# nv-tlabs/STRIVE

Measured on AMD Instinct MI355X. Metric: adv-optim agent*timesteps/sec (decoder fwd+bwd), higher is better.
Workload: dtype f32

## Files before the change

strive_amd/csrc/capi.hip:

```cpp
#include "common.h"
#include <stdarg.h>
#include <stddef.h>

static thread_local char g_err[512] = "";

void strive_set_error(const char* fmt, ...) {
    va_list ap;
    va_start(ap, fmt);
    vsnprintf(g_err, sizeof(g_err), fmt, ap);
    va_end(ap);
}

extern "C" const char* strive_last_error(void) { return g_err; }
extern "C" int strive_abi_version(void) { return STRIVE_ABI_VERSION; }

namespace {
struct OptionDesc { const char* name; size_t off; int def; int lo, hi; };
#define STRIVE_OPT(field, def, lo, hi) {#field, offsetof(StriveTuning, field), def, lo, hi}
const OptionDesc g_options[] = {
    STRIVE_OPT(cnn_small_batch, 96, 0, 1 << 20),
    STRIVE_OPT(cnn_chunk, 512, 8, 1024),
    STRIVE_OPT(cnn_tail_s, 0, 0, 4),
    STRIVE_OPT(conv_ws, 1, 0, 1),
    STRIVE_OPT(conv_wsx, 1, 0, 1),
    STRIVE_OPT(conv_ws_dbg, 0, 0, 255),
    STRIVE_OPT(scene_kernels, 1, 0, 1),
    STRIVE_OPT(scene_tiles, 1, 0, 1),
    STRIVE_OPT(scene_prof, 0, 0, 1),
    STRIVE_OPT(scene_split, 12, 0, 64),
    STRIVE_OPT(scene_fwd_k, -1, -1, 4),
    STRIVE_OPT(sweep_step, -1, -1, 4),
    STRIVE_OPT(train_overlap, 1, 0, 1),
    STRIVE_OPT(train_overlap_rows, 256, 1, 1 << 20),
    STRIVE_OPT(wgrad_atomics, 0, 0, 1),
    STRIVE_OPT(dgrad_igemm, 0, 0, 1),
    STRIVE_OPT(wgrad_igemm, 0, 0, 1),
    STRIVE_OPT(wgrad_tile, 0, 0, 1),
    STRIVE_OPT(wgrad_dbg, 0, 0, 255),
    STRIVE_OPT(planner_prof, 0, 0, 1),
    STRIVE_OPT(planner_dbg, 0, 0, 65535),
};
#undef STRIVE_OPT
constexpr int N_OPTIONS = (int)(sizeof(g_options) / sizeof(g_options[0]));
StriveTuning make_defaults() {
    StriveTuning t;
    for (int i = 0; i < N_OPTIONS; ++i) *reinterpret_cast<int*>(reinterpret_cast<char*>(&t) + g_options[i].off) = g_options[i].def;
    return t;
// ... 29 lines not shown
```

strive_amd/csrc/common.h:

```cpp
#pragma once
#include <hip/hip_runtime.h>
#include <atomic>
#include <stdint.h>
#include <stdio.h>
#include <string.h>
#include "../../include/strive_hip.h"

#define STRIVE_WAVE 64

void strive_set_error(const char* fmt, ...);

struct StriveTuning {
    int cnn_small_batch, cnn_chunk, cnn_tail_s, conv_ws, conv_wsx, conv_ws_dbg;
    int scene_kernels, scene_tiles, scene_prof, scene_split, scene_fwd_k, sweep_step;
    int train_overlap, train_overlap_rows;
    int wgrad_atomics, dgrad_igemm, wgrad_igemm, wgrad_tile, wgrad_dbg;
    int planner_prof;
    int planner_dbg;
};
StriveTuning& strive_tuning();

#define STRIVE_CHECK_ARG(cond, msg)                                   \
    do {                                                              \
        if (!(cond)) {                                                \
            strive_set_error("%s: %s", __func__, msg);                \
            return -1;                                                \
        }                                                             \
    } while (0)

#define STRIVE_CHECK_LAUNCH()                                                             \
    do {                                                                                  \
        hipError_t e__ = hipGetLastError();                                               \
        if (e__ != hipSuccess) {                                                          \
            strive_set_error("%s: kernel launch failed: %s", __func__, hipGetErrorString(e__)); \
            return -2;                                                                    \
        }                                                                                 \
// ... 86 lines not shown
```

strive_amd/csrc/map_cnn.hip:

```cpp
#include "common.h"
#include "crop_dev.h"
#include <type_traits>

typedef float f32x4 __attribute__((ext_vector_type(4)));
typedef float f32x16 __attribute__((ext_vector_type(16)));

#define GN_EPS 1e-5

struct GNStats { double sum, sq; };

__device__ __forceinline__ void gn_moments(const GNStats* __restrict__ st, int n, int nparts, double count, float& mean,
                                           float& rstd) {
    double s = 0.0, q = 0.0;
    for (int i = 0; i < nparts; ++i) {
        s += st[(size_t)n * nparts + i].sum;
        q += st[(size_t)n * nparts + i].sq;
    }
    const double m = s / count;
    double var = q / count - m * m;
    var = var < 0.0 ? 0.0 : var;
    mean = (float)m;
    rstd = (float)(1.0 / sqrt(var + GN_EPS));
}

// ... 210 lines not shown
    static constexpr int PT = PT_;
    static constexpr bool ROWS2 = ROWS2_;
    static constexpr int TILE_ROWS = ROWS2 ? 2 : 1;
    static constexpr int WGS_PER_CU = WGS_PER_CU_;
    static constexpr int NT = 256, NW = 4, TH = NW * PT * TILE_ROWS, TW = ROWS2 ? 16 : 32;
    static constexpr int CBW = CBW_, COUT_WG = 32 * CBW, CSPLIT = COUT / COUT_WG;
    static constexpr int PASS_CH = 8, NPASS = CIN / PASS_CH;
    static constexpr int ITH = 2 * TH + KS - 2, ITW = 2 * TW + KS - 2, HW = (ITW + 1) / 2;
    static constexpr int HALF_B = HW * 16, ROW_B = 2 * HALF_B, PIECE_B = ITH * ROW_B;
    static constexpr int NPIECE = 2;
    static constexpr int IN_B = (NPIECE * PIECE_B + 255) / 256 * 256;
    static constexpr int NKS = (KS * KS + 1) / 2;
    static constexpr int WSTEP_B = CBW * 2 * 64 * 16;
    static constexpr int TILES_X = (OH + TW - 1) / TW, TILES_Y = (OH + TH - 1) / TH;
    static constexpr int NPART_OUT = TILES_X * TILES_Y * CSPLIT;
    static constexpr int UNITS = ITH * ITW, UITERS = (UNITS + NT - 1) / NT;
    static constexpr size_t LDS_BYTES = (size_t)IN_B + 3 * WSTEP_B + (size_t)CIN * 8 + NW * 16 + 16 + COUT_WG * 4;
    static constexpr size_t WFRAG_BYTES = (size_t)NPASS * NKS * (COUT / 32) * 2048;
    static_assert(CIN % PASS_CH == 0 && COUT % COUT_WG == 0 && CIN <= NT, "channel tiling");
    static_assert(LDS_BYTES * WGS_PER_CU <= 160 * 1024, "LDS budget of the residency target");
    static_assert((KS == 5 && NKS == 13) || (KS == 3 && NKS == 5), "tap orders exist for 5x5 and 3x3 windows");
    static_assert(WSTEP_B == 16 * 128 * CBW && WSTEP_B / 16 <= NT, "weight step = one 16-byte piece for each of the first 128 CBW threads");
    static constexpr int W_UPFRONT = (WGS_PER_CU >= 3 && NKS > 8) ? 7 : NKS, W_LATE_AT = 2;
};

typedef float split_f32x2 __attribute__((ext_vector_type(2)));
typedef _Float16 split_f16x2v __attribute__((ext_vector_type(2)));
__device__ __forceinline__ void split_f16x2(const float v[8], uint4& p0, uint4& p1) {
    uint32_t h[4], l[4];
#pragma unroll
    for (int i = 0; i < 4; ++i) {
        const split_f32x2 v2 = {v[2 * i], v[2 * i + 1]};
        const split_f16x2v a = __builtin_convertvector(v2, split_f16x2v);
        const float r0 = v[2 * i] - (float)a[0];
        const float r1 = v[2 * i + 1] - (float)a[1];
        const split_f32x2 r2 = {r0, r1};
        const split_f16x2v c = __builtin_convertvector(r2, split_f16x2v);
        __builtin_memcpy(&h[i], &a, 4);
        __builtin_memcpy(&l[i], &c, 4);
    }
    p0 = make_uint4(h[0], h[1], h[2], h[3]);
    p1 = make_uint4(l[0], l[1], l[2], l[3]);
}

template <class Cfg, bool TIMING = false, int DBG = 0>
__global__ __launch_bounds__(Cfg::NT, Cfg::WGS_PER_CU) void conv_bf6_kernel(const float* __restrict__ in, const GNStats* __restrict__ st_in,
                                                                const float* __restrict__ gn_g, const float* __restrict__ gn_b,
                                                                const uint32_t* __restrict__ wfrag, const float* __restrict__ bias,
                                                                float* __restrict__ out, GNStats* __restrict__ st_out, int N,
                                                                float xscale, float unscale,
                                                                unsigned long long* __restrict__ tprof = nullptr) {
    long long tstamp[8];
    int nstamp = 0;
    auto stamp = [&]() { if (TIMING) tstamp[nstamp++] = clock64(); };
    stamp();
    constexpr int CIN = Cfg::CIN, COUT = Cfg::COUT, IH = Cfg::IH, OH = Cfg::OH, NT = Cfg::NT;
    constexpr int TH = Cfg::TH, TW = Cfg::TW, ITW = Cfg::ITW, PT = Cfg::PT;
    HIP_DYNAMIC_SHARED(float, smem)
    unsigned char* s_in = reinterpret_cast<unsigned char*>(smem);
    unsigned char* s_w = s_in + Cfg::IN_B;
    float* s_gn = (float*)(s_w + 3 * Cfg::WSTEP_B);
    double* s_red = (double*)(s_gn + 2 * CIN);
    float* s_mr = (float*)(s_red + 2 * Cfg::NW);
    float* s_bias = s_mr + 4;

    const int tid = threadIdx.x, lane = tid & 63, wave = tid >> 6;
    const int h = lane >> 5, j = lane & 31;
    int bx, by, n;
    {
        const unsigned T = gridDim.x * gridDim.y;
        const unsigned lin = blockIdx.x + gridDim.x * (blockIdx.y + gridDim.y * blockIdx.z);
        const unsigned q = lin >> 3, tile = q % T;
        n = (int)(8u * (q / T) + (lin & 7u));
        bx = (int)(tile % gridDim.x);
        by = (int)(tile / gridDim.x);
        if (n >= N) return;
    }
    const int tile_x = bx % Cfg::TILES_X, cb = bx / Cfg::TILES_X;
// ... 207 lines not shown
    const double lsum = wave_sum_d(dsum), lsq = wave_sum_d(dsq);
    if (lane == 0) { s_red[2 * wave] = lsum; s_red[2 * wave + 1] = lsq; }
    __syncthreads();
    if (tid == 0) {
        double a = 0.0, b = 0.0;
        for (int w = 0; w < Cfg::NW; ++w) { a += s_red[2 * w]; b += s_red[2 * w + 1]; }
        GNStats& o = st_out[(size_t)n * Cfg::NPART_OUT + (by * Cfg::TILES_X + tile_x) * Cfg::CSPLIT + cb];
        o.sum = a;
        o.sq = b;
    }
    stamp();
    if (TIMING && tid == 0) {
        atomicAdd(tprof, 1ull);
        for (int k = 0; k + 1 < nstamp; ++k) atomicAdd(tprof + 1 + k, (unsigned long long)(tstamp[k + 1] - tstamp[k]));
    }
}

template <class Cfg>
struct WsCfg {
    static constexpr int NCONS_W = 8, NT = 1024, NPROD = 512;
    static constexpr int UITERS = (Cfg::UNITS + NPROD - 1) / NPROD;
    static constexpr int W_B = Cfg::NPASS * Cfg::NKS * Cfg::WSTEP_B;
    static constexpr size_t LDS_BYTES = 2 * (size_t)Cfg::IN_B + W_B + 2 * (size_t)Cfg::CIN * 8 + 2 * 8 * 16 + 64 + Cfg::COUT * 4;
    static_assert(Cfg::CBW == 1 && Cfg::CSPLIT == 1 && Cfg::OUT_OCT && !Cfg::ROWS2 && Cfg::TH == NCONS_W, "built for conv2's shape");
    static_assert(LDS_BYTES <= 160 * 1024, "LDS budget");
};

template <class Cfg>
struct WsUnits {
    int t_begin, nunit;
    __device__ __forceinline__ void tile(int u, int& n, int& ty, int& tx, int& pass) const {
        constexpr int TPS = Cfg::TILES_X * Cfg::TILES_Y;
        const int t = t_begin + u / Cfg::NPASS;
        pass = u - (u / Cfg::NPASS) * Cfg::NPASS;
        n = t / TPS;
        const int r = t - n * TPS;
        tx = r / Cfg::TILES_Y;
        ty = r - tx * Cfg::TILES_Y;
    }
};

template <class Cfg>
__device__ __forceinline__ void ws_producer(const float* __restrict__ in, const GNStats* __restrict__ st_in, const float* __restrict__ gn_g,
                                         const float* __restrict__ gn_b, float xscale, unsigned char* s_in, float* s_gn,
                                         WsUnits<Cfg> un, int dbg, unsigned long long* __restrict__ tprof) {
    using W = WsCfg<Cfg>;
    constexpr int CIN = Cfg::CIN, IH = Cfg::IH, TH = Cfg::TH, TW = Cfg::TW, ITW = Cfg::ITW;
// ... 253 lines not shown
struct WxCfg {
    static constexpr int NCW = Cfg::NW, GW = Cfg::NW, NPW = NPW_, NT = 64 * (NCW + NPW + 1), NPROD = 64 * NPW;
    static constexpr int NSUB = Cfg::NKS > 7 ? 2 : 1;
    static constexpr int SUB_STEPS = (Cfg::NKS + NSUB - 1) / NSUB;
    static constexpr int WSUB_B = SUB_STEPS * Cfg::WSTEP_B;
    static constexpr int WCHUNKS = WSUB_B / 1024;
    static constexpr int UITERS = (Cfg::UNITS + NPROD - 1) / NPROD;
    static constexpr size_t LDS_BYTES = 2 * (size_t)Cfg::IN_B + 2 * (size_t)WSUB_B + 2 * (size_t)Cfg::CIN * 8 + 2 * GW * 16 + Cfg::COUT * 4 + 64;
    static_assert(Cfg::CSPLIT == 1 && Cfg::OUT_OCT && Cfg::NW == 4, "one workgroup computes all output channels of its tile");
    static_assert(LDS_BYTES <= 160 * 1024, "LDS budget");
    static_assert(NT <= 1024, "waves");
};

template <class Cfg, class W>
__device__ __forceinline__ void wx_producer(const float* __restrict__ in, const GNStats* __restrict__ st_in, const float* __restrict__ gn_g,
                                         const float* __restrict__ gn_b, float xscale, unsigned char* s_in, float* s_gn, WsUnits<Cfg> un,
                                         int dbg) {
    constexpr int CIN = Cfg::CIN, IH = Cfg::IH, TH = Cfg::TH, TW = Cfg::TW, ITW = Cfg::ITW;
    const int tid = threadIdx.x, lane = tid & 63;
    const int wave = __builtin_amdgcn_readfirstlane(tid >> 6);
    const int ptid = tid - 64 * W::NCW;
    const int nunit = un.nunit;
    float4 raw0[W::UITERS][2], raw1[W::UITERS][2];
    auto issue_loads = [&](int u, float4 (&raw)[W::UITERS][2]) {
        int n, ty, tx, pass;
        un.tile(u, n, ty, tx, pass);
        const float* in_n = in + (size_t)n * IH * IH * CIN;
        const int iy0 = 2 * ty * TH, ix0 = 2 * tx * TW;
#pragma unroll
        for (int k = 0; k < W::UITERS; ++k) {
            int idx = ptid + k * W::NPROD;
            idx = idx < Cfg::UNITS ? idx : Cfg::UNITS - 1;
            const int col = idx % ITW, r = idx / ITW;
            int iy = iy0 + r, ix = ix0 + col;
            iy = iy < IH ? iy : IH - 1;
            ix = ix < IH ? ix : IH - 1;
            const float4* src = reinterpret_cast<const float4*>(in_n + (((size_t)pass * IH + iy) * IH + ix) * 8);
            raw[k][0] = src[0];
            raw[k][1] = src[1];
        }
    };
    auto sample_moments = [&](int n) {
        double ps = 0.0, pq = 0.0;
        for (int i = lane; i < Cfg::NPART_IN; i += 64) {
            ps += st_in[(size_t)n * Cfg::NPART_IN + i].sum;
            pq += st_in[(size_t)n * Cfg::NPART_IN + i].sq;
        }
        ps = wave_sum_d(ps);
        pq = wave_sum_d(pq);
        const double cnt = (double)CIN * IH * IH;
        const double mu = ps / cnt;
        double var = pq / cnt - mu * mu;
        var = var < 0.0 ? 0.0 : var;
        const float mean = (float)mu, rstd = (float)(1.0 / sqrt(var + GN_EPS));
        if (lane < CIN) {
            const float sc = rstd * gn_g[lane];
            float* g = s_gn + (n & 1) * CIN * 2;
            g[2 * lane] = sc * xscale;
            g[2 * lane + 1] = (gn_b[lane] - mean * sc) * xscale;
        }
    };
    auto stage = [&](int u, const float4 (&raw)[W::UITERS][2], int chunk) {
        int n, ty, tx, pass;
        un.tile(u, n, ty, tx, pass);
        const int iy0 = 2 * ty * TH, ix0 = 2 * tx * TW;
        unsigned char* buf = s_in + (u & 1) * Cfg::IN_B;
        const float4* gn = reinterpret_cast<const float4*>(s_gn + (n & 1) * CIN * 2 + 2 * pass * Cfg::PASS_CH);
        const float4 g0 = gn[0], g1 = gn[1], g2 = gn[2], g3 = gn[3];
#pragma unroll
        for (int k = 0; k < W::UITERS; ++k) {
            if (chunk >= 0 && (k * W::NSUB) / W::UITERS != chunk) continue;
            const int idx = ptid + k * W::NPROD;
            if (idx < Cfg::UNITS) {
                const int col = idx % ITW, r = idx / ITW;
                const int iy = iy0 + r, ix = ix0 + col;
                float v[8];
#pragma unroll
                for (int e = 0; e < 8; ++e) v[e] = 0.f;
                if (iy < IH && ix < IH) {
                    const float4 a = raw[k][0], b = raw[k][1];
                    v[0] = fmaxf(fmaf(a.x, g0.x, g0.y), 0.f);
                    v[1] = fmaxf(fmaf(a.y, g0.z, g0.w), 0.f);
                    v[2] = fmaxf(fmaf(a.z, g1.x, g1.y), 0.f);
                    v[3] = fmaxf(fmaf(a.w, g1.z, g1.w), 0.f);
                    v[4] = fmaxf(fmaf(b.x, g2.x, g2.y), 0.f);
                    v[5] = fmaxf(fmaf(b.y, g2.z, g2.w), 0.f);
                    v[6] = fmaxf(fmaf(b.z, g3.x, g3.y), 0.f);
                    v[7] = fmaxf(fmaf(b.w, g3.z, g3.w), 0.f);
                }
                uint4 p0, p1;
                split_f16x2(v, p0, p1);
                unsigned char* dst = buf + r * Cfg::ROW_B + (col & 1) * Cfg::HALF_B + (col >> 1) * 16;
                *reinterpret_cast<uint4*>(dst) = p0;
                *reinterpret_cast<uint4*>(dst + Cfg::PIECE_B) = p1;
            }
        }
// ... 47 lines not shown
        for (int i = 0; i < W::WCHUNKS; ++i) w[i] = src[(i < nchunk ? i : nchunk - 1) * 64 + lane];
#pragma unroll
        for (int i = 0; i < W::WCHUNKS; ++i)
            if (i < nchunk) dst[i * 64 + lane] = w[i];
    };
    const int K = nunit * W::NSUB;
    __syncthreads();
    fill(0);
    __syncthreads();
    for (int k = 1; k <= K; ++k) {
        if (k < K && !(dbg & 8)) fill(k);
        __syncthreads();
    }
}

template <class Cfg, class W>
__device__ __forceinline__ void wx_consumer(const unsigned char* s_in, const unsigned char* s_w, double* s_red, const float* s_bias,
                                         float* __restrict__ out, GNStats* __restrict__ st_out, float unscale, WsUnits<Cfg> un, int dbg) {
    constexpr int COUT = Cfg::COUT, OH = Cfg::OH, TH = Cfg::TH, TW = Cfg::TW, NKS = Cfg::NKS, NPASS = Cfg::NPASS, PT = Cfg::PT, CBW = Cfg::CBW;
    const int tid = threadIdx.x, lane = tid & 63;
    const int wave = __builtin_amdgcn_readfirstlane(tid >> 6);
    const int h = lane >> 5, j = lane & 31;
    const int nunit = un.nunit;
    f32x16 acc[CBW][PT];
    const int gwave = wave;
    const int prow = Cfg::ROWS2 ? (j >> 4) : 0, pcol = Cfg::ROWS2 ? (j & 15) : j;
    const int lane_base = (2 * (Cfg::TILE_ROWS * PT * gwave + prow)) * Cfg::ROW_B + pcol * 16;

    auto matrix_sub = [&](int u, auto HC) {
        constexpr int HS = decltype(HC)::value;
        constexpr int S0 = HS * W::SUB_STEPS, S1 = (S0 + W::SUB_STEPS) < NKS ? (S0 + W::SUB_STEPS) : NKS;
        int n, ty, tx, pass;
        un.tile(u, n, ty, tx, pass);
        const unsigned char* buf = s_in + (u & 1) * Cfg::IN_B;
        const unsigned char* wbuf = s_w + ((u * W::NSUB + HS) & 1) * W::WSUB_B;
        if (pass == 0 && HS == 0) {
#pragma unroll
            for (int c = 0; c < CBW; ++c)
#pragma unroll
                for (int i = 0; i < PT; ++i)
#pragma unroll
                    for (int r = 0; r < 16; ++r) acc[c][i][r] = 0.f;
        }
        f16x8 fa[2][CBW][2], fb[2][PT][2];
        auto load_frags = [&](int t, int set) {
            int ky, kx;
            if (Cfg::KS == 5) {
                if (t < 10) { ky = t >> 1; kx = (t & 1) + 2 * h; }
                else { ky = 2 * (t - 10) + h; kx = 4; ky = ky > 4 ? 4 : ky; }
            } else {
                if (t < 3) { ky = t; kx = 2 * h; }
                else if (t == 3) { ky = h; kx = 1; }
                else { ky = 2; kx = 1; }
            }
            const int off = ky * Cfg::ROW_B + (kx & 1) * Cfg::HALF_B + (kx >> 1) * 16;
            const unsigned char* wb = wbuf + (t - S0) * Cfg::WSTEP_B + lane * 16;
#pragma unroll
            for (int c = 0; c < CBW; ++c)
#pragma unroll
                for (int pl = 0; pl < 2; ++pl) fa[set][c][pl] = *reinterpret_cast<const f16x8*>(wb + (c * 2 + pl) * 1024);
#pragma unroll
            for (int i = 0; i < PT; ++i)
#pragma unroll
                for (int pl = 0; pl < 2; ++pl)
                    fb[set][i][pl] = *reinterpret_cast<const f16x8*>(buf + pl * Cfg::PIECE_B + 2 * Cfg::TILE_ROWS * i * Cfg::ROW_B + lane_base + off);
        };
        load_frags(S0, 0);
#pragma unroll
        for (int s = S0; s < S1; ++s) {
            const int cur = (s - S0) & 1;
            if (s + 1 < S1) load_frags(s + 1, cur ^ 1);
            constexpr int TA[3] = {1, 0, 0}, TB[3] = {0, 1, 0};
#pragma unroll
            for (int term = 0; term < 3; ++term)
#pragma unroll
                for (int c = 0; c < CBW; ++c)
#pragma unroll
                    for (int i = 0; i < PT; ++i)
                        acc[c][i] = __builtin_amdgcn_mfma_f32_32x32x16_f16(fa[cur][c][TA[term]], fb[cur][i][TB[term]], acc[c][i], 0, 0, 0);
            if (s + 1 < S1) {
                constexpr int NRD = 2 * CBW + 2 * PT, NMF = 3 * PT * CBW;
#pragma unroll
                for (int q = 0; q < (NRD < NMF ? NRD : NMF); ++q) {
                    __builtin_amdgcn_sched_group_barrier(0x008, 1, 0);
                    __builtin_amdgcn_sched_group_barrier(0x100, 1, 0);
                }
                if (NMF > NRD) __builtin_amdgcn_sched_group_barrier(0x008, NMF - NRD, 0);
                if (NRD > NMF) __builtin_amdgcn_sched_group_barrier(0x100, NRD - NMF, 0);
            }
            __builtin_amdgcn_sched_barrier(0);
        }
    };
    double dsum = 0.0, dsq = 0.0;
    auto epilogue = [&](int u, int q0, int q1) {
        int n, ty, tx, pass;
        un.tile(u, n, ty, tx, pass);
        const int oy0 = ty * TH, ox0 = tx * TW;
        float* out_n = out + (size_t)n * COUT * OH * OH;
        constexpr int PLANE = OH * OH * 8;
        if (q0 == 0) { dsum = 0.0; dsq = 0.0; }
#pragma unroll
        for (int c = 0; c < CBW; ++c) {
#pragma unroll
            for (int i = 0; i < PT; ++i) {
                if (c * PT + i < q0 || c * PT + i >= q1) continue;
                float4 bv[4];
#pragma unroll
                for (int rg = 0; rg < 4; ++rg) bv[rg] = *reinterpret_cast<const float4*>(s_bias + c * 32 + 8 * rg + 4 * h);
                const int oy = oy0 + Cfg::TILE_ROWS * (PT * gwave + i) + prow, ox = ox0 + pcol;
                const bool valid = oy < OH && ox < OH;
                const int loff = (oy * OH + ox) * 8 + 4 * h;
                float fsum = 0.f, fsq = 0.f;
#pragma unroll
                for (int rg = 0; rg < 4; ++rg) {
                    float4 v;
                    v.x = fmaf(acc[c][i][4 * rg + 0], unscale, bv[rg].x);
                    v.y = fmaf(acc[c][i][4 * rg + 1], unscale, bv[rg].y);
                    v.z = fmaf(acc[c][i][4 * rg + 2], unscale, bv[rg].z);
                    v.w = fmaf(acc[c][i][4 * rg + 3], unscale, bv[rg].w);
                    if (valid) {
                        if (!(dbg & 64)) *reinterpret_cast<float4*>(out_n + (loff + (c * 4 + rg) * PLANE)) = v;
                        fsum += (v.x + v.y) + (v.z + v.w);
                        fsq = fmaf(v.x, v.x, fmaf(v.y, v.y, fmaf(v.z, v.z, fmaf(v.w, v.w, fsq))));
                    }
                }
                dsum += (double)fsum;
                dsq += (double)fsq;
            }
        }
        if (q1 == CBW * PT) {
            const double lsum = wave_sum_d(dsum), lsq = wave_sum_d(dsq);
            const int tl = (u / NPASS) & 1;
            if (lane == 0) { s_red[(tl * W::GW + gwave) * 2] = lsum; s_red[(tl * W::GW + gwave) * 2 + 1] = lsq; }
        }
    };
    auto publish_stats = [&](int u) {
        int n, ty, tx, pass;
        un.tile(u, n, ty, tx, pass);
        const int tl = (u / NPASS) & 1;
        double a = 0.0, b = 0.0;
        for (int w = 0; w < W::GW; ++w) { a += s_red[(tl * W::GW + w) * 2]; b += s_red[(tl * W::GW + w) * 2 + 1]; }
        GNStats& o = st_out[(size_t)n * Cfg::NPART_OUT + (ty * Cfg::TILES_X + tx)];
        o.sum = a;
        o.sq = b;
    };
    constexpr int NQ = CBW * PT;
    __syncthreads();
    __syncthreads();
    for (int u = 0; u < nunit; ++u) {
        if (!(dbg & 1)) matrix_sub(u, std::integral_constant<int, 0>());
        if (tid == 0 && u >= 1 && ((u - 1) % NPASS) == NPASS - 1) publish_stats(u - 1);
        if (W::NSUB == 1 && (u % NPASS) == NPASS - 1 && !(dbg & 16)) epilogue(u, 0, NQ);
        __syncthreads();
        if (W::NSUB == 2) {
            if (!(dbg & 1)) matrix_sub(u, std::integral_constant<int, W::NSUB - 1>());
            if ((u % NPASS) == NPASS - 1 && !(dbg & 16)) epilogue(u, 0, NQ);
            __syncthreads();
        }
    }
    if (tid == 0 && nunit >= 1 && ((nunit - 1) % NPASS) == NPASS - 1) publish_stats(nunit - 1);
}

template <class Cfg, int NPW = 7>
__global__ __launch_bounds__(64 * (Cfg::NW + NPW + 1), 1) void conv_wsx_kernel(const float* __restrict__ in, const GNStats* __restrict__ st_in,
                                                           const float* __restrict__ gn_g, const float* __restrict__ gn_b,
                                                           const uint32_t* __restrict__ wfrag, const float* __restrict__ bias,
                                                           float* __restrict__ out, GNStats* __restrict__ st_out, int N, float xscale,
                                                           float unscale, int dbg) {
    using W = WxCfg<Cfg, NPW>;
    HIP_DYNAMIC_SHARED(float, smem)
    unsigned char* s_in = reinterpret_cast<unsigned char*>(smem);
    unsigned char* s_w = s_in + 2 * Cfg::IN_B;
    float* s_gn = (float*)(s_w + 2 * W::WSUB_B);
    double* s_red = (double*)(s_gn + 2 * Cfg::CIN * 2);
    float* s_bias = (float*)(s_red + 2 * W::GW * 2);
    const int tid = threadIdx.x;
    const int wave = __builtin_amdgcn_readfirstlane(tid >> 6);
    const int total = N * Cfg::TILES_X * Cfg::TILES_Y;
    const int per = (total + (int)gridDim.x - 1) / (int)gridDim.x;
    WsUnits<Cfg> un;
    un.t_begin = (int)blockIdx.x * per;
// ... 248 lines not shown
        o.sum = a;
        o.sq = b;
    }
}

template <class Cfg>
static int launch_bf6s(const float* in, const GNStats* st_in, const float* g, const float* b, const uint32_t* wfrag,
                       const float* bias, float* out, GNStats* st_out, int N, float xscale, float wscale, hipStream_t stream) {
    dim3 grid(((N + Cfg::S - 1) / Cfg::S) * Cfg::CSPLIT);
    static PerDeviceOnce once;
    const int dev = once.device();
    if (!once.is_done(dev)) {
        hipFuncSetAttribute((const void*)conv_bf6s_kernel<Cfg>, hipFuncAttributeMaxDynamicSharedMemorySize, (int)Cfg::LDS_BYTES);
        once.set_done(dev);
    }
    hipLaunchKernelGGL(conv_bf6s_kernel<Cfg>, grid, dim3(Cfg::NT), Cfg::LDS_BYTES, stream, in, st_in, g, b, wfrag, bias, out,
                       st_out, N, xscale, 1.0f / (xscale * wscale));
    return 0;
}

typedef BfCfg<16, 32, 5, 125, 61, l1b::NPART, true, 2, 3> Bf2;
typedef BfCfg<32, 64, 5, 61, 29, Bf2::NPART_OUT, true, 2, 2, false, 2> Bf3;
typedef BfCfg<64, 64, 3, 29, 14, Bf3::NPART_OUT, true, 2, 2, true, 2> Bf4;
typedef BfCfg<32, 64, 5, 61, 29, Bf2::NPART_OUT, true, 1, 2, false, 1> Bf3s;
typedef BfCfg<64, 64, 3, 29, 14, Bf3s::NPART_OUT, true, 1, 2, true, 1> Bf4s;
typedef BfsCfg<64, 128, 14, 6, 7, Bf4::NPART_OUT, true, 2, 2> Bfs5;
typedef BfsCfg<128, 128, 6, 2, 32, Bfs5::NPART_OUT, false, 1, 2> Bfs6;


template <class Cfg>
static int launch_ws(const float* in, const GNStats* st_in, const float* g, const float* b, const uint32_t* wfrag,
                     const float* bias, float* out, GNStats* st_out, int N, float xscale, float wscale, hipStream_t stream,
                     unsigned long long* tprof = nullptr) {
    using W = WsCfg<Cfg>;
    static PerDeviceOnce once;
    const int dev = once.device();
    if (!once.is_done(dev)) {
        hipFuncSetAttribute((const void*)conv_ws_kernel<Cfg>, hipFuncAttributeMaxDynamicSharedMemorySize, (int)W::LDS_BYTES);
        int v = 0;
        if (!(hipDeviceGetAttribute(&v, hipDeviceAttributeMultiprocessorCount, dev) == hipSuccess && v > 0)) v = 256;
        once.value[dev].store(v, std::memory_order_relaxed);
        once.set_done(dev);
    }
    const int ncu = once.value[dev].load(std::memory_order_relaxed);
    const int total = N * Cfg::TILES_X * Cfg::TILES_Y;
    const int grid = total < ncu ? total : ncu;
// ... 191 lines not shown
        dim3 g1(l1b::TILES_Y, n <= small_batch ? l1b::TILES_X : 1, n);
        const int tail_s = tail_force ? tail_force : (n <= CNN_TAIL_ONE_SAMPLE ? 1 : 2);
        if (map) {
            hipLaunchKernelGGL(conv1b_kernel<true>, g1, dim3(C1_NT), 0, stream, mp, pos + (size_t)n0 * 4, m, s, mapix + n0,
                               (const uint8_t*)nullptr, cnn->w1_frag, 1.0f / cnn->wscale[0], (const float*)cnn->b[0], act[0], st[0]);
        } else {
            hipLaunchKernelGGL(conv1b_kernel<false>, g1, dim3(C1_NT), 0, stream, mp, (const float*)nullptr, m, s,
                               (const int32_t*)nullptr, crop + (size_t)n0 * 4 * 256 * 256, cnn->w1_frag, 1.0f / cnn->wscale[0],
                               (const float*)cnn->b[0], act[0], st[0]);
        }
        const bool conv_ws = strive_tuning().conv_ws != 0;
        if (conv_ws && !cnn->conv2_plain)
            launch_ws<Bf2>(act[0], st[0], cnn->gn_g[0], cnn->gn_b[0], cnn->w2_frag, cnn->b[1], act[1], st[1], n, cnn->xscale[1], cnn->wscale[1], stream);
        else
            launch_bf6<Bf2>(act[0], st[0], cnn->gn_g[0], cnn->gn_b[0], cnn->w2_frag, cnn->b[1], act[1], st[1], n, cnn->xscale[1], cnn->wscale[1], stream);
        if (!keep_tail_activations && !keep && n <= small_batch) {
            launch_bf6<Bf3s>(act[1], st[1], cnn->gn_g[1], cnn->gn_b[1], cnn->w3_frag, cnn->b[2], act[2], st[2], n, cnn->xscale[2], cnn->wscale[2], stream);
            launch_bf6<Bf4s>(act[2], st[2], cnn->gn_g[2], cnn->gn_b[2], cnn->w4_frag, cnn->b[3], act[3], st[3], n, cnn->xscale[3], cnn->wscale[3], stream);
            launch_cnn_tail(cnn, act[3], st[3], Bf4s::NPART_OUT, feat + (size_t)n0 * 64, n, stream, nullptr, tail_s);
            continue;
        }
        const bool conv_wsx = strive_tuning().conv_wsx != 0;
        if (conv_wsx && !cnn->conv2_plain) {
            launch_wsx<Bf3>(act[1], st[1], cnn->gn_g[1], cnn->gn_b[1], cnn->w3_frag, cnn->b[2], act[2], st[2], n, cnn->xscale[2], cnn->wscale[2], stream);
            launch_wsx<Bf4>(act[2], st[2], cnn->gn_g[2], cnn->gn_b[2], cnn->w4_frag, cnn->b[3], act[3], st[3], n, cnn->xscale[3], cnn->wscale[3], stream);
        } else {
            launch_bf6<Bf3>(act[1], st[1], cnn->gn_g[1], cnn->gn_b[1], cnn->w3_frag, cnn->b[2], act[2], st[2], n, cnn->xscale[2], cnn->wscale[2], stream);
            launch_bf6<Bf4>(act[2], st[2], cnn->gn_g[2], cnn->gn_b[2], cnn->w4_frag, cnn->b[3], act[3], st[3], n, cnn->xscale[3], cnn->wscale[3], stream);
        }
        if (!keep_tail_activations) {
            launch_cnn_tail(cnn, act[3], st[3], NPARTS[3], feat + (size_t)n0 * 64, n, stream, nullptr, tail_s, keep ? &tk : nullptr);
            continue;
        }
        launch_bf6s<Bfs5>(act[3], st[3], cnn->gn_g[3], cnn->gn_b[3], cnn->w5_frag, cnn->b[4], act[4], st[4], n, cnn->xscale[4], cnn->wscale[4], stream);
        launch_bf6s<Bfs6>(act[4], st[4], cnn->gn_g[4], cnn->gn_b[4], cnn->w6_frag, cnn->b[5], act[5], st[5], n, cnn->xscale[5], cnn->wscale[5], stream);
        hipLaunchKernelGGL(fc_kernel, dim3((n + 3) / 4), dim3(256), 0, stream, act[5], st[5], cnn->gn_g[5], cnn->gn_b[5],
                           cnn->fc_wt, cnn->fc_b, feat + (size_t)n0 * 64, n);
    }
    STRIVE_CHECK_LAUNCH();
    return 0;
}

extern "C" int strive_map_cnn_fwd(const StriveMap* map, const StriveCNN* cnn, const float* pos,
                                  const float* pos_mean4_host, const float* pos_std4_host, const int32_t* mapix, int32_t N,
                                  float* feat, void* ws, size_t ws_bytes, strive_stream_t stream) {
    STRIVE_CHECK_ARG(map && cnn && pos && mapix && feat && ws && pos_mean4_host && pos_std4_host, "null argument");
    STRIVE_CHECK_ARG(map->C == 4 && map->L == 256 && map->Wc == 256, "the HIP map CNN supports the default 4x256x256 crop only");
    return cnn_run(map, cnn, pos, pos_mean4_host, pos_std4_host, mapix, nullptr, N, feat, ws, ws_bytes, (hipStream_t)stream);
// ... 76 lines not shown
                if (dbg == 1) { STRIVE_DBG_LAUNCH(Bf2, 1, act[0], st[0], cnn->gn_g[0], cnn->gn_b[0], cnn->w2_frag, cnn->b[1], act[1], st[1], 1); }
                if (dbg == 2) { STRIVE_DBG_LAUNCH(Bf2, 2, act[0], st[0], cnn->gn_g[0], cnn->gn_b[0], cnn->w2_frag, cnn->b[1], act[1], st[1], 1); }
                if (dbg == 3) { STRIVE_DBG_LAUNCH(Bf2, 3, act[0], st[0], cnn->gn_g[0], cnn->gn_b[0], cnn->w2_frag, cnn->b[1], act[1], st[1], 1); }
                if (dbg == 4) { STRIVE_DBG_LAUNCH(Bf2, 4, act[0], st[0], cnn->gn_g[0], cnn->gn_b[0], cnn->w2_frag, cnn->b[1], act[1], st[1], 1); }
            } else {
                if (dbg == 1) { STRIVE_DBG_LAUNCH(Bf3, 1, act[1], st[1], cnn->gn_g[1], cnn->gn_b[1], cnn->w3_frag, cnn->b[2], act[2], st[2], 2); }
                if (dbg == 2) { STRIVE_DBG_LAUNCH(Bf3, 2, act[1], st[1], cnn->gn_g[1], cnn->gn_b[1], cnn->w3_frag, cnn->b[2], act[2], st[2], 2); }
                if (dbg == 3) { STRIVE_DBG_LAUNCH(Bf3, 3, act[1], st[1], cnn->gn_g[1], cnn->gn_b[1], cnn->w3_frag, cnn->b[2], act[2], st[2], 2); }
                if (dbg == 4) { STRIVE_DBG_LAUNCH(Bf3, 4, act[1], st[1], cnn->gn_g[1], cnn->gn_b[1], cnn->w3_frag, cnn->b[2], act[2], st[2], 2); }
            }
#undef STRIVE_DBG_LAUNCH
            break;
        }
        case 1: launch_bf6<Bf2>(act[0], st[0], cnn->gn_g[0], cnn->gn_b[0], cnn->w2_frag, cnn->b[1], act[1], st[1], N, cnn->xscale[1], cnn->wscale[1], stream); break;
        case 51: launch_ws<Bf2>(act[0], st[0], cnn->gn_g[0], cnn->gn_b[0], cnn->w2_frag, cnn->b[1], act[1], st[1], N, cnn->xscale[1], cnn->wscale[1], stream); break;
        case 81: {
            unsigned long long* tp = reinterpret_cast<unsigned long long*>(feat);
            hipMemsetAsync(tp, 0, 64, stream);
            launch_ws<Bf2>(act[0], st[0], cnn->gn_g[0], cnn->gn_b[0], cnn->w2_frag, cnn->b[1], act[1], st[1], N, cnn->xscale[1], cnn->wscale[1], stream, tp);
            break;
        }
        case 52: launch_wsx<Bf3>(act[1], st[1], cnn->gn_g[1], cnn->gn_b[1], cnn->w3_frag, cnn->b[2], act[2], st[2], N, cnn->xscale[2], cnn->wscale[2], stream); break;
        case 53: launch_wsx<Bf4>(act[2], st[2], cnn->gn_g[2], cnn->gn_b[2], cnn->w4_frag, cnn->b[3], act[3], st[3], N, cnn->xscale[3], cnn->wscale[3], stream); break;
        case 2: launch_bf6<Bf3>(act[1], st[1], cnn->gn_g[1], cnn->gn_b[1], cnn->w3_frag, cnn->b[2], act[2], st[2], N, cnn->xscale[2], cnn->wscale[2], stream); break;
        case 3: launch_bf6<Bf4>(act[2], st[2], cnn->gn_g[2], cnn->gn_b[2], cnn->w4_frag, cnn->b[3], act[3], st[3], N, cnn->xscale[3], cnn->wscale[3], stream); break;
        case 4: launch_bf6s<Bfs5>(act[3], st[3], cnn->gn_g[3], cnn->gn_b[3], cnn->w5_frag, cnn->b[4], act[4], st[4], N, cnn->xscale[4], cnn->wscale[4], stream); break;
        case 5: launch_bf6s<Bfs6>(act[4], st[4], cnn->gn_g[4], cnn->gn_b[4], cnn->w6_frag, cnn->b[5], act[5], st[5], N, cnn->xscale[5], cnn->wscale[5], stream); break;
        case 7: launch_cnn_tail(cnn, act[3], st[3], NPARTS[3], feat, N, stream, nullptr, N <= CNN_TAIL_ONE_SAMPLE ? 1 : 2); break;
        case 27: {
            unsigned long long* tp = reinterpret_cast<unsigned long long*>(act[4]);
            hipMemsetAsync(tp, 0, 64, stream);
            launch_cnn_tail(cnn, act[3], st[3], NPARTS[3], feat, N, stream, tp);
            hipMemcpyAsync(feat, tp, 64, hipMemcpyDeviceToDevice, stream);
            break;
        }
        default:
            hipLaunchKernelGGL(fc_kernel, dim3((N + 3) / 4), dim3(256), 0, stream, act[5], st[5], cnn->gn_g[5], cnn->gn_b[5],
                               cnn->fc_wt, cnn->fc_b, feat, N);
    }
    STRIVE_CHECK_LAUNCH();
    return 0;
}

#include "map_cnn_bwd.h"
```

Before: 727,400.

## Tile conv3/conv4 output as flat pixel bands to cut wasted MFMA tiles

Adds a flat tiling for the conv3 and conv4 warp-specialized kernels. Output pixels are numbered linearly and grouped into bands of 32-pixel MFMA tiles, replacing square 2D tiles that leave partly empty tiles at the edges. Per-band staging windows, per-lane gather offsets and specializations for partially live tiles are added, and the new form is on by default. The cost is irregular LDS addressing per lane, extra template instances and a larger input staging area.

```diff
diff --git a/strive_amd/csrc/capi.hip b/strive_amd/csrc/capi.hip
--- a/strive_amd/csrc/capi.hip
+++ b/strive_amd/csrc/capi.hip
@@ -23,6 +23,7 @@
     STRIVE_OPT(cnn_tail_s, 0, 0, 4),
     STRIVE_OPT(conv_ws, 1, 0, 1),
     STRIVE_OPT(conv_wsx, 1, 0, 1),
+    STRIVE_OPT(conv_flat, 3, 0, 3),
     STRIVE_OPT(conv_ws_dbg, 0, 0, 255),
     STRIVE_OPT(scene_kernels, 1, 0, 1),
     STRIVE_OPT(scene_tiles, 1, 0, 1),
diff --git a/strive_amd/csrc/common.h b/strive_amd/csrc/common.h
--- a/strive_amd/csrc/common.h
+++ b/strive_amd/csrc/common.h
@@ -11,7 +11,7 @@
 void strive_set_error(const char* fmt, ...);
 
 struct StriveTuning {
-    int cnn_small_batch, cnn_chunk, cnn_tail_s, conv_ws, conv_wsx, conv_ws_dbg;
+    int cnn_small_batch, cnn_chunk, cnn_tail_s, conv_ws, conv_wsx, conv_flat, conv_ws_dbg;
     int scene_kernels, scene_tiles, scene_prof, scene_split, scene_fwd_k, sweep_step;
     int train_overlap, train_overlap_rows;
     int wgrad_atomics, dgrad_igemm, wgrad_igemm, wgrad_tile, wgrad_dbg;
diff --git a/strive_amd/csrc/map_cnn.hip b/strive_amd/csrc/map_cnn.hip
--- a/strive_amd/csrc/map_cnn.hip
+++ b/strive_amd/csrc/map_cnn.hip
@@ -256,6 +256,43 @@
     static_assert((KS == 5 && NKS == 13) || (KS == 3 && NKS == 5), "tap orders exist for 5x5 and 3x3 windows");
     static_assert(WSTEP_B == 16 * 128 * CBW && WSTEP_B / 16 <= NT, "weight step = one 16-byte piece for each of the first 128 CBW threads");
     static constexpr int W_UPFRONT = (WGS_PER_CU >= 3 && NKS > 8) ? 7 : NKS, W_LATE_AT = 2;
+    static constexpr bool FLAT = false;
+};
+
+constexpr int flat_band_y0(int b, int band_p, int oh) { return b * band_p / oh; }
+constexpr int flat_band_y1(int b, int band_p, int oh) { return (((b + 1) * band_p < oh * oh ? (b + 1) * band_p : oh * oh) - 1) / oh; }
+constexpr int flat_max_band_rows(int nband, int band_p, int oh) {
+    int m = 0;
+    for (int b = 0; b < nband; ++b) {
+        const int r = flat_band_y1(b, band_p, oh) - flat_band_y0(b, band_p, oh) + 1;
+        m = r > m ? r : m;
+    }
+    return m;
+}
+template <class B>
+struct FlatCfg : B {
+    static constexpr bool FLAT = true;
+    static constexpr int PIX = B::OH * B::OH;
+    static constexpr int TILES_S = (PIX + 31) / 32;
+    static constexpr int BAND_T = B::NW * B::PT, BAND_P = 32 * BAND_T;
+    static constexpr int NBAND = (TILES_S + BAND_T - 1) / BAND_T;
+    static constexpr int ITH = 2 * (flat_max_band_rows(NBAND, BAND_P, B::OH) - 1) + B::KS, ITW = B::IH, HW = (ITW + 1) / 2;
+    static constexpr int HALF_B = HW * 16, ROW_B = 2 * HALF_B, PIECE_B = ITH * ROW_B;
+    static constexpr int IN_B = (B::NPIECE * PIECE_B + 255) / 256 * 256;
+    static constexpr int TILES_X = 1, TILES_Y = NBAND;
+    static constexpr int NPART_OUT = NBAND;
+    static constexpr int UNITS = ITH * ITW;
+    static constexpr int band_iy0(int b) { return 2 * flat_band_y0(b, BAND_P, B::OH); }
+    static constexpr int band_units(int b) {
+        return (2 * (flat_band_y1(b, BAND_P, B::OH) - flat_band_y0(b, BAND_P, B::OH)) + B::KS) * B::IH;
+    }
+    static constexpr int live_tiles(int b, int w) {
+        const int r = TILES_S - b * BAND_T - w;
+        return r <= 0 ? 0 : ((r + B::NW - 1) / B::NW < B::PT ? (r + B::NW - 1) / B::NW : B::PT);
+    }
+    static_assert(B::CSPLIT == 1 && B::CBW == 2 && B::PT == 2, "built for conv3 / conv4 on conv_wsx_kernel");
+    static_assert(NPART_OUT == B::NPART_OUT, "the tiled form's statistics slots: the next layer reads either form");
+    static_assert(2 * (B::OH - 1) + B::KS <= B::IH, "valid convolution: every staged row exists");
 };
 
 typedef float split_f32x2 __attribute__((ext_vector_type(2)));
@@ -288,6 +325,7 @@
     int nstamp = 0;
     auto stamp = [&]() { if (TIMING) tstamp[nstamp++] = clock64(); };
     stamp();
+    static_assert(!Cfg::FLAT, "the flat tiling exists on conv_wsx_kernel only");
     constexpr int CIN = Cfg::CIN, COUT = Cfg::COUT, IH = Cfg::IH, OH = Cfg::OH, NT = Cfg::NT;
     constexpr int TH = Cfg::TH, TW = Cfg::TW, ITW = Cfg::ITW, PT = Cfg::PT;
     HIP_DYNAMIC_SHARED(float, smem)
@@ -541,7 +579,7 @@
     static constexpr int UITERS = (Cfg::UNITS + NPROD - 1) / NPROD;
     static constexpr int W_B = Cfg::NPASS * Cfg::NKS * Cfg::WSTEP_B;
     static constexpr size_t LDS_BYTES = 2 * (size_t)Cfg::IN_B + W_B + 2 * (size_t)Cfg::CIN * 8 + 2 * 8 * 16 + 64 + Cfg::COUT * 4;
-    static_assert(Cfg::CBW == 1 && Cfg::CSPLIT == 1 && Cfg::OUT_OCT && !Cfg::ROWS2 && Cfg::TH == NCONS_W, "built for conv2's shape");
+    static_assert(Cfg::CBW == 1 && Cfg::CSPLIT == 1 && Cfg::OUT_OCT && !Cfg::ROWS2 && !Cfg::FLAT && Cfg::TH == NCONS_W, "built for conv2's shape");
     static_assert(LDS_BYTES <= 160 * 1024, "LDS budget");
 };
 
@@ -841,15 +879,27 @@
     const int ptid = tid - 64 * W::NCW;
     const int nunit = un.nunit;
     float4 raw0[W::UITERS][2], raw1[W::UITERS][2];
+    auto window = [&](int u, int& n, int& pass, int& iy0, int& ix0, int& units) {
+        int ty, tx;
+        un.tile(u, n, ty, tx, pass);
+        if constexpr (Cfg::FLAT) {
+            iy0 = Cfg::band_iy0(ty);
+            ix0 = 0;
+            units = Cfg::band_units(ty);
+        } else {
+            iy0 = 2 * ty * TH;
+            ix0 = 2 * tx * TW;
+            units = Cfg::UNITS;
+        }
+    };
     auto issue_loads = [&](int u, float4 (&raw)[W::UITERS][2]) {
-        int n, ty, tx, pass;
-        un.tile(u, n, ty, tx, pass);
+        int n, pass, iy0, ix0, units;
+        window(u, n, pass, iy0, ix0, units);
         const float* in_n = in + (size_t)n * IH * IH * CIN;
-        const int iy0 = 2 * ty * TH, ix0 = 2 * tx * TW;
 #pragma unroll
         for (int k = 0; k < W::UITERS; ++k) {
             int idx = ptid + k * W::NPROD;
-            idx = idx < Cfg::UNITS ? idx : Cfg::UNITS - 1;
+            idx = idx < units ? idx : units - 1;
             const int col = idx % ITW, r = idx / ITW;
             int iy = iy0 + r, ix = ix0 + col;
             iy = iy < IH ? iy : IH - 1;
@@ -880,9 +930,8 @@
         }
     };
     auto stage = [&](int u, const float4 (&raw)[W::UITERS][2], int chunk) {
-        int n, ty, tx, pass;
-        un.tile(u, n, ty, tx, pass);
-        const int iy0 = 2 * ty * TH, ix0 = 2 * tx * TW;
+        int n, pass, iy0, ix0, units;
+        window(u, n, pass, iy0, ix0, units);
         unsigned char* buf = s_in + (u & 1) * Cfg::IN_B;
         const float4* gn = reinterpret_cast<const float4*>(s_gn + (n & 1) * CIN * 2 + 2 * pass * Cfg::PASS_CH);
         const float4 g0 = gn[0], g1 = gn[1], g2 = gn[2], g3 = gn[3];
@@ -890,7 +939,7 @@
         for (int k = 0; k < W::UITERS; ++k) {
             if (chunk >= 0 && (k * W::NSUB) / W::UITERS != chunk) continue;
             const int idx = ptid + k * W::NPROD;
-            if (idx < Cfg::UNITS) {
+            if (idx < units) {
                 const int col = idx % ITW, r = idx / ITW;
                 const int iy = iy0 + r, ix = ix0 + col;
                 float v[8];
@@ -984,13 +1033,35 @@
     const int wave = __builtin_amdgcn_readfirstlane(tid >> 6);
     const int h = lane >> 5, j = lane & 31;
     const int nunit = un.nunit;
-    f32x16 acc[CBW][PT];
     const int gwave = wave;
     const int prow = Cfg::ROWS2 ? (j >> 4) : 0, pcol = Cfg::ROWS2 ? (j & 15) : j;
-    const int lane_base = (2 * (Cfg::TILE_ROWS * PT * gwave + prow)) * Cfg::ROW_B + pcol * 16;
-
-    auto matrix_sub = [&](int u, auto HC) {
-        constexpr int HS = decltype(HC)::value;
+    const int lane_base = Cfg::FLAT ? 0 : (2 * (Cfg::TILE_ROWS * PT * gwave + prow)) * Cfg::ROW_B + pcol * 16;
+    int tile_base[PT];
+    int nlive = PT;
+#pragma unroll
+    for (int i = 0; i < PT; ++i) tile_base[i] = lane_base + 2 * Cfg::TILE_ROWS * i * Cfg::ROW_B;
+    auto flat_pixel = [&](int b, int i) {
+        if constexpr (Cfg::FLAT) return b * Cfg::BAND_P + 32 * (i * Cfg::NW + gwave) + j;
+        else return 0;
+    };
+    auto band_geometry = [&](int u) {
+        if constexpr (Cfg::FLAT) {
+            int n, ty, tx, pass;
+            un.tile(u, n, ty, tx, pass);
+            nlive = Cfg::live_tiles(ty, gwave);
+            const int iy0 = Cfg::band_iy0(ty);
+#pragma unroll
+            for (int i = 0; i < PT; ++i) {
+                int p = flat_pixel(ty, i);
+                p = p < Cfg::PIX ? p : Cfg::PIX - 1;
+                const int oy = p / OH, ox = p - oy * OH;
+                tile_base[i] = (2 * oy - iy0) * Cfg::ROW_B + ox * 16;
+            }
+        }
+    };
+
+    auto matrix_sub = [&](int u, auto HC, auto NC, auto& acc) {
+        constexpr int HS = decltype(HC)::value, NPT = decltype(NC)::value;
         constexpr int S0 = HS * W::SUB_STEPS, S1 = (S0 + W::SUB_STEPS) < NKS ? (S0 + W::SUB_STEPS) : NKS;
         int n, ty, tx, pass;
         un.tile(u, n, ty, tx, pass);
@@ -1000,7 +1071,7 @@
 #pragma unroll
             for (int c = 0; c < CBW; ++c)
 #pragma unroll
-                for (int i = 0; i < PT; ++i)
+                for (int i = 0; i < NPT; ++i)
 #pragma unroll
                     for (int r = 0; r < 16; ++r) acc[c][i][r] = 0.f;
         }
@@ -1022,10 +1093,10 @@
 #pragma unroll
                 for (int pl = 0; pl < 2; ++pl) fa[set][c][pl] = *reinterpret_cast<const f16x8*>(wb + (c * 2 + pl) * 1024);
 #pragma unroll
-            for (int i = 0; i < PT; ++i)
+            for (int i = 0; i < NPT; ++i)
 #pragma unroll
                 for (int pl = 0; pl < 2; ++pl)
-                    fb[set][i][pl] = *reinterpret_cast<const f16x8*>(buf + pl * Cfg::PIECE_B + 2 * Cfg::TILE_ROWS * i * Cfg::ROW_B + lane_base + off);
+                    fb[set][i][pl] = *reinterpret_cast<const f16x8*>(buf + pl * Cfg::PIECE_B + tile_base[i] + off);
         };
         load_frags(S0, 0);
 #pragma unroll
@@ -1038,10 +1109,10 @@
 #pragma unroll
                 for (int c = 0; c < CBW; ++c)
 #pragma unroll
-                    for (int i = 0; i < PT; ++i)
+                    for (int i = 0; i < NPT; ++i)
                         acc[c][i] = __builtin_amdgcn_mfma_f32_32x32x16_f16(fa[cur][c][TA[term]], fb[cur][i][TB[term]], acc[c][i], 0, 0, 0);
             if (s + 1 < S1) {
-                constexpr int NRD = 2 * CBW + 2 * PT, NMF = 3 * PT * CBW;
+                constexpr int NRD = 2 * CBW + 2 * NPT, NMF = 3 * NPT * CBW;
 #pragma unroll
                 for (int q = 0; q < (NRD < NMF ? NRD : NMF); ++q) {
                     __builtin_amdgcn_sched_group_barrier(0x008, 1, 0);
@@ -1054,7 +1125,8 @@
         }
     };
     double dsum = 0.0, dsq = 0.0;
-    auto epilogue = [&](int u, int q0, int q1) {
+    auto epilogue = [&](int u, int q0, int q1, auto NC, auto& acc) {
+        constexpr int NPT = decltype(NC)::value;
         int n, ty, tx, pass;
         un.tile(u, n, ty, tx, pass);
         const int oy0 = ty * TH, ox0 = tx * TW;
@@ -1065,13 +1137,21 @@
         for (int c = 0; c < CBW; ++c) {
 #pragma unroll
             for (int i = 0; i < PT; ++i) {
-                if (c * PT + i < q0 || c * PT + i >= q1) continue;
+                if (c * PT + i < q0 || c * PT + i >= q1 || i >= NPT) continue;
                 float4 bv[4];
 #pragma unroll
                 for (int rg = 0; rg < 4; ++rg) bv[rg] = *reinterpret_cast<const float4*>(s_bias + c * 32 + 8 * rg + 4 * h);
-                const int oy = oy0 + Cfg::TILE_ROWS * (PT * gwave + i) + prow, ox = ox0 + pcol;
-                const bool valid = oy < OH && ox < OH;
-                const int loff = (oy * OH + ox) * 8 + 4 * h;
+                bool valid;
+                int loff;
+                if constexpr (Cfg::FLAT) {
+                    const int p = flat_pixel(ty, i);
+                    valid = p < Cfg::PIX;
+                    loff = p * 8 + 4 * h;
+                } else {
+                    const int oy = oy0 + Cfg::TILE_ROWS * (PT * gwave + i) + prow, ox = ox0 + pcol;
+                    valid = oy < OH && ox < OH;
+                    loff = (oy * OH + ox) * 8 + 4 * h;
+                }
                 float fsum = 0.f, fsq = 0.f;
 #pragma unroll
                 for (int rg = 0; rg < 4; ++rg) {
@@ -1109,16 +1189,25 @@
     constexpr int NQ = CBW * PT;
     __syncthreads();
     __syncthreads();
-    for (int u = 0; u < nunit; ++u) {
-        if (!(dbg & 1)) matrix_sub(u, std::integral_constant<int, 0>());
-        if (tid == 0 && u >= 1 && ((u - 1) % NPASS) == NPASS - 1) publish_stats(u - 1);
-        if (W::NSUB == 1 && (u % NPASS) == NPASS - 1 && !(dbg & 16)) epilogue(u, 0, NQ);
-        __syncthreads();
-        if (W::NSUB == 2) {
-            if (!(dbg & 1)) matrix_sub(u, std::integral_constant<int, W::NSUB - 1>());
-            if ((u % NPASS) == NPASS - 1 && !(dbg & 16)) epilogue(u, 0, NQ);
+    auto tile_units = [&](int t0, auto NC) {
+        f32x16 acc[CBW][decltype(NC)::value > 0 ? decltype(NC)::value : 1];
+        for (int u = t0; u < t0 + NPASS; ++u) {
+            if (!(dbg & 1) && decltype(NC)::value > 0) matrix_sub(u, std::integral_constant<int, 0>(), NC, acc);
+            if (tid == 0 && u >= 1 && ((u - 1) % NPASS) == NPASS - 1) publish_stats(u - 1);
+            if (W::NSUB == 1 && (u % NPASS) == NPASS - 1 && !(dbg & 16)) epilogue(u, 0, NQ, NC, acc);
             __syncthreads();
-        }
+            if (W::NSUB == 2) {
+                if (!(dbg & 1) && decltype(NC)::value > 0) matrix_sub(u, std::integral_constant<int, W::NSUB - 1>(), NC, acc);
+                if ((u % NPASS) == NPASS - 1 && !(dbg & 16)) epilogue(u, 0, NQ, NC, acc);
+                __syncthreads();
+            }
+        }
+    };
+    for (int t0 = 0; t0 < nunit; t0 += NPASS) {
+        band_geometry(t0);
+        if (!Cfg::FLAT || nlive == PT) tile_units(t0, std::integral_constant<int, PT>());
+        else if (Cfg::FLAT && PT > 1 && nlive == 1) tile_units(t0, std::integral_constant<int, (Cfg::FLAT && PT > 1 ? 1 : PT)>());
+        else tile_units(t0, std::integral_constant<int, (Cfg::FLAT ? 0 : PT)>());
     }
     if (tid == 0 && nunit >= 1 && ((nunit - 1) % NPASS) == NPASS - 1) publish_stats(nunit - 1);
 }
@@ -1413,6 +1502,11 @@
 typedef BfCfg<16, 32, 5, 125, 61, l1b::NPART, true, 2, 3> Bf2;
 typedef BfCfg<32, 64, 5, 61, 29, Bf2::NPART_OUT, true, 2, 2, false, 2> Bf3;
 typedef BfCfg<64, 64, 3, 29, 14, Bf3::NPART_OUT, true, 2, 2, true, 2> Bf4;
+typedef FlatCfg<Bf3> Bf3f;
+typedef FlatCfg<Bf4> Bf4f;
+static_assert(Bf3f::ITH == 23 && Bf3f::IN_B == 45824 && WxCfg<Bf3f>::WSUB_B == 28672 && WxCfg<Bf3f>::LDS_BYTES == 149952 &&
+              Bf4f::ITH == 29 && Bf4f::IN_B == 27904 && WxCfg<Bf4f>::WSUB_B == 20480 && WxCfg<Bf4f>::LDS_BYTES == 98240,
+              "LDS arithmetic of the flat conv3 / conv4 (within the 160 KB of a CU: WxCfg)");
 typedef BfCfg<32, 64, 5, 61, 29, Bf2::NPART_OUT, true, 1, 2, false, 1> Bf3s;
 typedef BfCfg<64, 64, 3, 29, 14, Bf3s::NPART_OUT, true, 1, 2, true, 1> Bf4s;
 typedef BfsCfg<64, 128, 14, 6, 7, Bf4::NPART_OUT, true, 2, 2> Bfs5;
@@ -1650,8 +1744,15 @@
         }
         const bool conv_wsx = strive_tuning().conv_wsx != 0;
         if (conv_wsx && !cnn->conv2_plain) {
-            launch_wsx<Bf3>(act[1], st[1], cnn->gn_g[1], cnn->gn_b[1], cnn->w3_frag, cnn->b[2], act[2], st[2], n, cnn->xscale[2], cnn->wscale[2], stream);
-            launch_wsx<Bf4>(act[2], st[2], cnn->gn_g[2], cnn->gn_b[2], cnn->w4_frag, cnn->b[3], act[3], st[3], n, cnn->xscale[3], cnn->wscale[3], stream);
+            const int flat = strive_tuning().conv_flat;
+            if (flat & 1)
+                launch_wsx<Bf3f>(act[1], st[1], cnn->gn_g[1], cnn->gn_b[1], cnn->w3_frag, cnn->b[2], act[2], st[2], n, cnn->xscale[2], cnn->wscale[2], stream);
+            else
+                launch_wsx<Bf3>(act[1], st[1], cnn->gn_g[1], cnn->gn_b[1], cnn->w3_frag, cnn->b[2], act[2], st[2], n, cnn->xscale[2], cnn->wscale[2], stream);
+            if (flat & 2)
+                launch_wsx<Bf4f>(act[2], st[2], cnn->gn_g[2], cnn->gn_b[2], cnn->w4_frag, cnn->b[3], act[3], st[3], n, cnn->xscale[3], cnn->wscale[3], stream);
+            else
+                launch_wsx<Bf4>(act[2], st[2], cnn->gn_g[2], cnn->gn_b[2], cnn->w4_frag, cnn->b[3], act[3], st[3], n, cnn->xscale[3], cnn->wscale[3], stream);
         } else {
             launch_bf6<Bf3>(act[1], st[1], cnn->gn_g[1], cnn->gn_b[1], cnn->w3_frag, cnn->b[2], act[2], st[2], n, cnn->xscale[2], cnn->wscale[2], stream);
             launch_bf6<Bf4>(act[2], st[2], cnn->gn_g[2], cnn->gn_b[2], cnn->w4_frag, cnn->b[3], act[3], st[3], n, cnn->xscale[3], cnn->wscale[3], stream);
@@ -1774,6 +1875,8 @@
         }
         case 52: launch_wsx<Bf3>(act[1], st[1], cnn->gn_g[1], cnn->gn_b[1], cnn->w3_frag, cnn->b[2], act[2], st[2], N, cnn->xscale[2], cnn->wscale[2], stream); break;
         case 53: launch_wsx<Bf4>(act[2], st[2], cnn->gn_g[2], cnn->gn_b[2], cnn->w4_frag, cnn->b[3], act[3], st[3], N, cnn->xscale[3], cnn->wscale[3], stream); break;
+        case 62: launch_wsx<Bf3f>(act[1], st[1], cnn->gn_g[1], cnn->gn_b[1], cnn->w3_frag, cnn->b[2], act[2], st[2], N, cnn->xscale[2], cnn->wscale[2], stream); break;
+        case 63: launch_wsx<Bf4f>(act[2], st[2], cnn->gn_g[2], cnn->gn_b[2], cnn->w4_frag, cnn->b[3], act[3], st[3], N, cnn->xscale[3], cnn->wscale[3], stream); break;
         case 2: launch_bf6<Bf3>(act[1], st[1], cnn->gn_g[1], cnn->gn_b[1], cnn->w3_frag, cnn->b[2], act[2], st[2], N, cnn->xscale[2], cnn->wscale[2], stream); break;
         case 3: launch_bf6<Bf4>(act[2], st[2], cnn->gn_g[2], cnn->gn_b[2], cnn->w4_frag, cnn->b[3], act[3], st[3], N, cnn->xscale[3], cnn->wscale[3], stream); break;
         case 4: launch_bf6s<Bfs5>(act[3], st[3], cnn->gn_g[3], cnn->gn_b[3], cnn->w5_frag, cnn->b[4], act[4], st[4], N, cnn->xscale[4], cnn->wscale[4], stream); break;
```

Result: no change. 733,500, median of 6 (+0.8%).
